# jbush001/RustNetworkStack

Measured on AMD Instinct MI355X. Metric: GiB/s device-resident Internet checksum, 1500B-packet batches, 1/2/4/8 GPUs, higher is better.
Workload: dtype u8

## Files before the change

include/rns_checksum.h:

```cpp
#ifndef RNS_CHECKSUM_H
#define RNS_CHECKSUM_H

#include <stddef.h>
#include <stdint.h>

#ifdef __cplusplus
extern "C" {
#endif

#define RNS_ABI_VERSION 1

#define RNS_OK            0
#define RNS_E_INVALID    (-1)
#define RNS_E_EMPTY      (-2)
#define RNS_E_BOUNDS     (-3)
#define RNS_E_NODEVICE   (-4)
#define RNS_E_ORDER      (-5)
#define RNS_E_TOOLARGE   (-6)
#define RNS_E_IO         (-7)
#define RNS_E_HIP_BASE   (-1000)

#define RNS_FLAG_COMPLEMENT 0x1u
#define RNS_FLAG_CHAIN_RUNS 0x2u
#define RNS_FLAG_CHAIN_TX_PACKED 0x4u

typedef struct rns_iovec {
    const uint8_t *base;
    size_t len;
} rns_iovec;

typedef struct rns_ipaddr {
    uint32_t version;
    uint8_t bytes[16];
} rns_ipaddr;


int32_t rns_compute_ones_comp(uint16_t in_checksum, const uint8_t *slice, size_t len);

int32_t rns_compute_checksum(const uint8_t *slice, size_t len);

int32_t rns_compute_buffer_ones_comp(uint16_t initial_sum, const rns_iovec *frags, size_t nfrags);

int32_t rns_compute_pseudo_header_checksum(const rns_ipaddr *source_ip, const rns_ipaddr *dest_ip,
                                           uint64_t length, uint8_t protocol);


int rns_csum_batch_dev(const uint8_t *d_arena, uint64_t arena_bytes, const uint64_t *d_off,
                       const uint32_t *d_len, const uint16_t *d_seed, uint16_t *d_out, uint32_t n,
                       uint32_t flags, uint32_t len_hint, uint32_t *d_bad, void *stream);

int rns_csum_batch_dev_off32(const uint8_t *d_arena, uint64_t arena_bytes, const uint32_t *d_off32,
                             const uint32_t *d_len, const uint16_t *d_seed, uint16_t *d_out, uint32_t n,
                             uint32_t flags, uint32_t len_hint, uint32_t *d_bad, void *stream);

int rns_csum_batch_packed_dev(const uint8_t *d_arena, uint64_t arena_bytes, const uint64_t *d_blk_off,
                              const uint16_t *d_len16, uint32_t align_log2, const uint16_t *d_seed, uint16_t *d_out,
                              uint32_t n, uint32_t flags, uint32_t len_hint, uint32_t *d_bad, void *stream);

int rns_packed_layout(const uint16_t *len16, uint64_t n, uint32_t align_log2, uint64_t first_off, uint64_t *blk_off,
                      uint64_t *off, uint64_t *end);

int rns_csum_batch_strided_dev(const uint8_t *d_arena, uint64_t arena_bytes, uint64_t first_off,
                               uint64_t stride, uint32_t len, const uint16_t *d_seed, uint16_t *d_out,
                               uint32_t n, uint32_t flags, uint32_t *d_bad, void *stream);

#define RNS_CHAIN_MAX_PACKETS (0xFFFFFFFFu - 512u)
int rns_csum_chain_dev(const uint8_t *d_arena, uint64_t arena_bytes, const uint64_t *d_frag_off,
                       const uint32_t *d_frag_len, uint32_t n_frags, const uint32_t *d_first,
                       const uint16_t *d_seed, uint16_t *d_out, uint32_t n_pkts, uint32_t flags,
                       uint32_t frag_len_hint, uint16_t *d_frag_sums, uint32_t *d_bad, void *stream);

int rns_csum_chain_fill_dev(uint8_t *d_arena, uint64_t arena_bytes, const uint64_t *d_frag_off,
                            const uint32_t *d_frag_len, uint32_t n_frags, const uint32_t *d_first,
                            const uint16_t *d_seed, const uint16_t *d_field, uint32_t field_off, uint16_t *d_out,
                            uint32_t n_pkts, uint32_t flags, uint32_t frag_len_hint, uint32_t *d_bad, void *stream);

int rns_csum_fill_dev(uint8_t *d_arena, uint64_t arena_bytes, const uint64_t *d_off, const uint32_t *d_len,
                      const uint16_t *d_seed, const uint16_t *d_field, uint32_t field_off, uint16_t *d_out,
                      uint32_t n, uint32_t flags, uint32_t *d_bad, void *stream);

int rns_csum_fill_packed_dev(uint8_t *d_arena, uint64_t arena_bytes, const uint64_t *d_blk_off, const uint16_t *d_len16,
                             uint32_t align_log2, const uint16_t *d_seed, const uint16_t *d_field, uint32_t field_off,
                             uint16_t *d_out, uint32_t n, uint32_t flags, uint32_t len_hint, uint32_t *d_bad,
                             void *stream);

#define RNS_RX_IP_OK          0x01u
#define RNS_RX_L4_OK          0x02u
#define RNS_RX_L4_UNCHECKED   0x04u
#define RNS_RX_FRAGMENT       0x08u
#define RNS_RX_UNKNOWN_PROTO  0x10u
#define RNS_RX_ACCEPT         0x40u
#define RNS_RX_MALFORMED      0x80u
int rns_rx_verify_dev(const uint8_t *d_arena, uint64_t arena_bytes, const uint64_t *d_off, const uint32_t *d_len,
                      uint32_t n, const uint8_t *local_ipv4, const uint8_t *local_ipv6, uint8_t *d_status,
                      uint16_t *d_l4_sum, void *stream);

int rns_rx_verify_packed_dev(const uint8_t *d_arena, uint64_t arena_bytes, const uint64_t *d_blk_off,
                             const uint16_t *d_len16, uint32_t align_log2, uint32_t n, const uint8_t *local_ipv4,
                             const uint8_t *local_ipv6, uint8_t *d_status, uint16_t *d_l4_sum, void *stream);

int rns_rx_verify_strided_dev(const uint8_t *d_arena, uint64_t arena_bytes, uint64_t first_off, uint64_t stride,
                              const uint16_t *d_len16, uint32_t n, const uint8_t *local_ipv4, const uint8_t *local_ipv6,
                              uint8_t *d_status, uint16_t *d_l4_sum, void *stream);

#define RNS_TX_IP_FILLED      0x01u
#define RNS_TX_L4_FILLED      0x02u
// ... 84 lines not shown
```

rustnetworkstack_amd/_lib.py:

```python
from __future__ import annotations

import ctypes
import os
import threading

PKG_DIR = os.path.dirname(os.path.abspath(__file__))
LIB_PATH = os.environ.get("RNS_CHECKSUM_LIB") or os.path.join(PKG_DIR, "librns_checksum.so")

RNS_OK = 0
RNS_E_INVALID = -1
RNS_E_EMPTY = -2
RNS_E_BOUNDS = -3
RNS_E_NODEVICE = -4
RNS_E_ORDER = -5
RNS_E_TOOLARGE = -6
RNS_E_IO = -7
RNS_E_HIP_BASE = -1000
RNS_FLAG_COMPLEMENT = 0x1
RNS_FLAG_CHAIN_RUNS = 0x2
RNS_FLAG_CHAIN_TX_PACKED = 0x4
RNS_CHAIN_MAX_PACKETS = 0xFFFFFFFF - 512
RNS_IO_MAX_FRAGS = 8
RNS_RX_IP_OK = 0x01
RNS_RX_L4_OK = 0x02
RNS_RX_L4_UNCHECKED = 0x04
RNS_RX_FRAGMENT = 0x08
RNS_RX_UNKNOWN_PROTO = 0x10
RNS_RX_ACCEPT = 0x40
RNS_RX_MALFORMED = 0x80
RNS_TX_IP_FILLED = 0x01
RNS_TX_L4_FILLED = 0x02
RNS_TX_MALFORMED = 0x80

EXPORTED_SYMBOLS = (
    "rns_compute_ones_comp",
    "rns_compute_checksum",
    "rns_compute_buffer_ones_comp",
    "rns_compute_pseudo_header_checksum",
    "rns_csum_batch_dev",
    "rns_csum_batch_dev_off32",
    "rns_csum_batch_packed_dev",
    "rns_packed_layout",
    "rns_csum_batch_strided_dev",
    "rns_csum_batch_dev_cfg",
    "rns_csum_chain_dev",
    "rns_csum_chain_fill_dev",
    "rns_csum_fill_dev",
    "rns_csum_fill_packed_dev",
    "rns_rx_verify_dev",
    "rns_rx_verify_packed_dev",
    "rns_rx_verify_strided_dev",
    "rns_tx_fill_dev",
    "rns_tx_fill_packed_dev",
    "rns_tx_fill_chain_dev",
    "rns_tx_fill_chain_packed_dev",
    "rns_tx_chain_packed_layout",
    "rns_host_ctx_create",
    "rns_host_ctx_destroy",
    "rns_csum_batch_host",
    "rns_multi_ctx_create",
    "rns_multi_ctx_destroy",
    "rns_csum_batch_multi_host",
    "rns_csum_batch_multi_dev",
    "rns_io_recv_batch",
    "rns_io_send_batch",
    "rns_io_send_batch_chain",
    "rns_io_recv_batch_packed",
    "rns_host_alloc",
    "rns_host_free",
    "rns_fill_splitmix64_dev",
    "rns_abi_version",
    "rns_strerror",
    "rns_build_info",
    "rns_csum_shape_name",
    "rns_device_count",
)


class ChecksumLibraryMissing(RuntimeError):
    """librns_checksum.so is not built: run __graft_entry__.build() (or `make`)."""


class ChecksumError(RuntimeError):
    def __init__(self, status: int, what: str):
        self.status = status
        super().__init__(f"{what}: {strerror(status)} (status {status})")


class RnsIovec(ctypes.Structure):
    _fields_ = [("base", ctypes.c_void_p), ("len", ctypes.c_size_t)]


class RnsIpAddr(ctypes.Structure):
    _fields_ = [("version", ctypes.c_uint32), ("bytes", ctypes.c_uint8 * 16)]


class RnsDevBatch(ctypes.Structure):
    _fields_ = [("device", ctypes.c_int), ("d_arena", ctypes.c_void_p), ("arena_bytes", ctypes.c_uint64),
                ("d_off", ctypes.c_void_p), ("d_len", ctypes.c_void_p), ("d_seed", ctypes.c_void_p),
                ("d_out", ctypes.c_void_p), ("n", ctypes.c_uint32), ("len_hint", ctypes.c_uint32),
                ("d_bad", ctypes.c_void_p), ("stream", ctypes.c_void_p)]


_LIB = None
_LOCK = threading.Lock()

_vp, _u8, _u16, _u32, _u64, _i32, _int, _sz = (
    ctypes.c_void_p, ctypes.c_uint8, ctypes.c_uint16, ctypes.c_uint32, ctypes.c_uint64,
    ctypes.c_int32, ctypes.c_int, ctypes.c_size_t)

_SIGNATURES = {
    "rns_compute_ones_comp": (_i32, [_u16, _vp, _sz]),
    "rns_compute_checksum": (_i32, [_vp, _sz]),
    "rns_compute_buffer_ones_comp": (_i32, [_u16, ctypes.POINTER(RnsIovec), _sz]),
    "rns_compute_pseudo_header_checksum": (_i32, [ctypes.POINTER(RnsIpAddr), ctypes.POINTER(RnsIpAddr), _u64, _u8]),
    "rns_csum_batch_dev": (_int, [_vp, _u64, _vp, _vp, _vp, _vp, _u32, _u32, _u32, _vp, _vp]),
    "rns_csum_batch_dev_off32": (_int, [_vp, _u64, _vp, _vp, _vp, _vp, _u32, _u32, _u32, _vp, _vp]),
    "rns_csum_batch_packed_dev": (_int, [_vp, _u64, _vp, _vp, _u32, _vp, _vp, _u32, _u32, _u32, _vp, _vp]),
    "rns_packed_layout": (_int, [_vp, _u64, _u32, _u64, _vp, _vp, ctypes.POINTER(_u64)]),
    "rns_csum_batch_strided_dev": (_int, [_vp, _u64, _u64, _u64, _u32, _vp, _vp, _u32, _u32, _vp, _vp]),
    "rns_csum_batch_dev_cfg": (_int, [_vp, _u64, _vp, _vp, _vp, _vp, _u32, _u32, _u32, _u32, _u32, _u32, _vp, _vp]),
    "rns_csum_chain_dev": (_int, [_vp, _u64, _vp, _vp, _u32, _vp, _vp, _vp, _u32, _u32, _u32, _vp, _vp, _vp]),
    "rns_csum_chain_fill_dev": (_int, [_vp, _u64, _vp, _vp, _u32, _vp, _vp, _vp, _u32, _vp, _u32, _u32, _u32, _vp,
                                       _vp]),
    "rns_csum_fill_dev": (_int, [_vp, _u64, _vp, _vp, _vp, _vp, _u32, _vp, _u32, _u32, _vp, _vp]),
    "rns_csum_fill_packed_dev": (_int, [_vp, _u64, _vp, _vp, _u32, _vp, _vp, _u32, _vp, _u32, _u32, _u32, _vp, _vp]),
    "rns_rx_verify_dev": (_int, [_vp, _u64, _vp, _vp, _u32, _vp, _vp, _vp, _vp, _vp]),
    "rns_rx_verify_packed_dev": (_int, [_vp, _u64, _vp, _vp, _u32, _u32, _vp, _vp, _vp, _vp, _vp]),
    "rns_rx_verify_strided_dev": (_int, [_vp, _u64, _u64, _u64, _vp, _u32, _vp, _vp, _vp, _vp, _vp]),
    "rns_tx_fill_dev": (_int, [_vp, _u64, _vp, _vp, _u32, _vp, _vp]),
    "rns_tx_fill_packed_dev": (_int, [_vp, _u64, _vp, _vp, _u32, _u32, _vp, _u32, _vp]),
    "rns_tx_fill_chain_dev": (_int, [_vp, _u64, _vp, _vp, _u32, _vp, _u32, _vp, _vp]),
    "rns_tx_fill_chain_packed_dev": (_int, [_vp, _u64, _vp, _vp, _vp, _vp, _u32, _u32, _vp, _vp]),
    "rns_tx_chain_packed_layout": (_int, [_vp, _vp, _u64, _u32, _u64, _u64, _vp, _vp, _vp, _vp,
                                          ctypes.POINTER(_u64), ctypes.POINTER(_u64)]),
    "rns_host_ctx_create": (_int, [_int, _u64, _u32, ctypes.POINTER(_vp)]),
    "rns_host_ctx_destroy": (_int, [_vp]),
    "rns_csum_batch_host": (_int, [_vp, _vp, _u64, _vp, _vp, _vp, _vp, _u32, _u32]),
    "rns_multi_ctx_create": (_int, [ctypes.POINTER(ctypes.c_int), _u32, _u64, _u32, ctypes.POINTER(_vp)]),
    "rns_multi_ctx_destroy": (_int, [_vp]),
    "rns_csum_batch_multi_host": (_int, [_vp, _vp, _u64, _vp, _vp, _vp, _vp, _u32, _u32]),
    "rns_csum_batch_multi_dev": (_int, [ctypes.POINTER(RnsDevBatch), _u32, _u32]),
    "rns_io_recv_batch": (_int, [_int, _vp, _u64, _u32, _vp, _vp, _int]),
    "rns_io_send_batch": (_int, [_int, _vp, _vp, _vp, _u32]),
    "rns_io_send_batch_chain": (_int, [_int, _vp, _vp, _vp, _vp, _u32]),
    "rns_io_recv_batch_packed": (_int, [_int, _vp, _u64, _u32, _u32, _vp, _vp, ctypes.POINTER(_u64), _int]),
    "rns_host_alloc": (_int, [_u64, ctypes.POINTER(_vp)]),
    "rns_host_free": (_int, [_vp]),
    "rns_fill_splitmix64_dev": (_int, [_vp, _u64, _u64, _vp]),
    "rns_abi_version": (_int, []),
    "rns_strerror": (ctypes.c_char_p, [_int]),
    "rns_build_info": (ctypes.c_char_p, []),
    "rns_csum_shape_name": (ctypes.c_char_p, [_u32]),
    "rns_device_count": (_int, []),
}


def load() -> ctypes.CDLL:
    global _LIB
    with _LOCK:
        if _LIB is None:
            try:
                import torch
            except ImportError:
                pass
            if not os.path.exists(LIB_PATH):
                raise ChecksumLibraryMissing(f"{LIB_PATH} not found; run __graft_entry__.build()")
            lib = ctypes.CDLL(LIB_PATH)
            for name, (res, args) in _SIGNATURES.items():
                fn = getattr(lib, name)
# ... 17 lines not shown
```

rustnetworkstack_amd/batch.py:

```python
from __future__ import annotations

import ctypes

import numpy as np
import torch

from . import _lib


def _require_cuda(t: torch.Tensor, name: str, dtypes) -> None:
    if not isinstance(t, torch.Tensor):
        raise TypeError(f"{name} must be a torch.Tensor")
    if t.device.type != "cuda":
        raise ValueError(f"{name} must be on a GPU device (got {t.device}); there is no CPU fallback")
    if t.dtype not in dtypes:
        raise TypeError(f"{name} dtype {t.dtype} not in {dtypes}")
    if not t.is_contiguous():
        raise ValueError(f"{name} must be contiguous")


_U16 = (torch.uint16, torch.int16)


def _rx_outputs(dev: torch.device, n: int, status, l4_sum, inputs):
# ... 125 lines not shown
        seed_ptr = None
        if seed is not None:
            _require_cuda(seed, "seed", _U16)
            if seed.numel() != n or seed.device != dev:
                raise ValueError("seed must have one entry per packet on the arena's device")
            seed_ptr = seed.data_ptr()
        if out is None:
            out = torch.empty(n, dtype=torch.uint16, device=dev)
        else:
            _require_cuda(out, "out", _U16)
            if out.numel() != n or out.device != dev:
                raise ValueError("out must have one entry per packet on the arena's device")
        bad_ptr = _bad_ptr(bad, arena.device)
        lib = _lib.load()
        self._keep = (arena, blk_off, len16, seed, out, bad)
        self.out, self.n, self.device = out, n, dev
        self._fn = lib.rns_csum_batch_packed_dev
        self._args = (arena.data_ptr(), arena.numel(), blk_off.data_ptr(), len16.data_ptr(), int(align_log2),
                      seed_ptr, out.data_ptr(), n, _lib.RNS_FLAG_COMPLEMENT if complement else 0, int(len_hint),
                      bad_ptr, _stream_handle(dev))

    def __call__(self) -> torch.Tensor:
        if self.n:
            if torch.cuda.current_device() != self.device.index:
                with torch.cuda.device(self.device):
                    st = self._fn(*self._args)
            else:
                st = self._fn(*self._args)
            if st != _lib.RNS_OK:
                raise _lib.ChecksumError(st, "rns_csum_batch_packed_dev")
        return self.out


def csum_batch_packed(arena: torch.Tensor, blk_off: torch.Tensor, len16: torch.Tensor,
                      seed: torch.Tensor | None = None, *, align_log2: int = 4, complement: bool = False,
                      out: torch.Tensor | None = None, len_hint: int = 0,
                      bad: torch.Tensor | None = None) -> torch.Tensor:
    _require_cuda(arena, "arena", (torch.uint8,))
    with torch.cuda.device(arena.device):
        return PackedBatch(arena, blk_off, len16, seed, align_log2=align_log2, complement=complement, out=out,
                           len_hint=len_hint, bad=bad)()


def csum_batch(arena: torch.Tensor, off: torch.Tensor, length: torch.Tensor, seed: torch.Tensor | None = None,
               *, complement: bool = False, out: torch.Tensor | None = None, len_hint: int = 0,
               bad: torch.Tensor | None = None, shape: tuple[int, int, int, int] | None = None,
               compact: bool = False) -> torch.Tensor:
    _require_cuda(arena, "arena", (torch.uint8,))
    with torch.cuda.device(arena.device):
        return PreparedBatch(arena, off, length, seed, complement=complement, out=out, len_hint=len_hint, bad=bad,
                             shape=shape, compact=compact)()


class StridedBatch:

    def __init__(self, arena: torch.Tensor, n: int, stride: int, length: int, *, first_off: int = 0,
                 seed: torch.Tensor | None = None, complement: bool = False,
                 out: torch.Tensor | None = None, bad: torch.Tensor | None = None):
        _require_cuda(arena, "arena", (torch.uint8,))
        dev = arena.device
        if n < 0 or n >= 2 ** 32 or stride < 0 or not 0 <= length < 2 ** 32 or first_off < 0:
            raise ValueError("n, stride, length and first_off must be non-negative (n, length < 2^32)")
        seed_ptr = None
        if seed is not None:
            _require_cuda(seed, "seed", _U16)
            if seed.numel() != n or seed.device != dev:
                raise ValueError("seed must have one entry per packet on the arena's device")
            seed_ptr = seed.data_ptr()
        if out is None:
            out = torch.empty(n, dtype=torch.uint16, device=dev)
        else:
            _require_cuda(out, "out", _U16)
            if out.numel() != n or out.device != dev:
                raise ValueError("out must have one entry per packet on the arena's device")
        bad_ptr = _bad_ptr(bad, arena.device)
        lib = _lib.load()
        self._keep = (arena, seed, out, bad)
        self.out, self.n, self.device = out, int(n), dev
        self._fn = lib.rns_csum_batch_strided_dev
        self._args = (arena.data_ptr(), arena.numel(), int(first_off), int(stride), int(length), seed_ptr,
                      out.data_ptr(), int(n), _lib.RNS_FLAG_COMPLEMENT if complement else 0, bad_ptr,
                      _stream_handle(dev))

    def __call__(self) -> torch.Tensor:
        if self.n:
            if torch.cuda.current_device() != self.device.index:
                with torch.cuda.device(self.device):
                    st = self._fn(*self._args)
            else:
                st = self._fn(*self._args)
            if st != _lib.RNS_OK:
                raise _lib.ChecksumError(st, "rns_csum_batch_strided_dev")
        return self.out


def csum_batch_strided(arena: torch.Tensor, n: int, stride: int, length: int, *, first_off: int = 0,
                       seed: torch.Tensor | None = None, complement: bool = False,
                       out: torch.Tensor | None = None, bad: torch.Tensor | None = None) -> torch.Tensor:
    _require_cuda(arena, "arena", (torch.uint8,))
    with torch.cuda.device(arena.device):
        return StridedBatch(arena, n, stride, length, first_off=first_off, seed=seed, complement=complement,
                            out=out, bad=bad)()


def csum_chain(arena: torch.Tensor, frag_off: torch.Tensor, frag_len: torch.Tensor, first: torch.Tensor,
               seed: torch.Tensor | None = None, *, complement: bool = False, out: torch.Tensor | None = None,
# ... 557 lines not shown
```

rustnetworkstack_amd/csrc/k_packed.hip:

```cpp
#include "rns_launch.hpp"

#ifndef RNS_ROWS_DEEP_FROM
#define RNS_ROWS_DEEP_FROM 1024u
#endif

namespace rns {

#ifndef RNS_RX_ROWS_D
#define RNS_RX_ROWS_D 8
#endif
int launch_stream_rx(const CsumArgs &a, hipStream_t st)
{
    const dim3 grid(static_cast<uint32_t>((static_cast<uint64_t>(a.n) + 63) / 64)), block(64);
    constexpr bool NT = RNS_STREAM_NT != 0;
    const bool ack = a.arena_bytes / a.n <= 128, buf = buf_records(a) < kOobOffset;
    if (ack && buf)
        hipLaunchKernelGGL((csum_stream_kernel<NT, true>), grid, block, 0, st, a);
    else if (ack)
        hipLaunchKernelGGL((csum_stream_kernel<NT, false>), grid, block, 0, st, a);
    else if (buf)
        hipLaunchKernelGGL((csum_rows_rx_kernel<NT, true, RNS_RX_ROWS_D>), grid, block, 0, st, a);
    else
        hipLaunchKernelGGL((csum_rows_rx_kernel<NT, false, RNS_RX_ROWS_D>), grid, block, 0, st, a);
    return hip_status(hipGetLastError());
}

int dispatch_packed(const CsumArgs &a, const Shape &sh, hipStream_t st)
{
    const bool nt = (sh.variant & 2u) != 0, buf = buf_records(a) < kOobOffset;
    const bool tiny = (sh.variant & ~16u) == 3u && sh.G == 4u && sh.U == 1u;
    if (a.align_mask >= 15u && !tiny) {
        constexpr bool NT = RNS_STREAM_NT != 0;
        const dim3 grid(static_cast<uint32_t>((static_cast<uint64_t>(a.n) + 63) / 64)), block(64);
        if (a.len_hint >= RNS_ROWS_DEEP_FROM) {
            if (buf)
                hipLaunchKernelGGL((csum_rows_kernel<NT, true, 16>), grid, block, 0, st, a);
            else
                hipLaunchKernelGGL((csum_rows_kernel<NT, false, 16>), grid, block, 0, st, a);
        } else {
            if (buf)
                hipLaunchKernelGGL((csum_rows_kernel<NT, true, 8>), grid, block, 0, st, a);
            else
                hipLaunchKernelGGL((csum_rows_kernel<NT, false, 8>), grid, block, 0, st, a);
        }
        return hip_status(hipGetLastError());
    }
    const uint64_t batches = (static_cast<uint64_t>(a.n) + 63) / 64;
    const uint64_t wpb = ((sh.variant & 4u) ? kMixedBlock<false> : kBlock) / 64;
    uint64_t blocks = (batches + wpb - 1) / wpb;
    if (sh.max_blocks != 0 && blocks > sh.max_blocks)
        blocks = sh.max_blocks;
    const dim3 grid(static_cast<uint32_t>(blocks)), block((sh.variant & 4u) ? kMixedBlock<false> : kBlock);
    if (sh.variant & 4u) {
        if (nt && buf)
            hipLaunchKernelGGL((csum_mixed_kernel<false, true, true, false, false, false, true>), grid, block, 0, st, a);
        else if (nt)
            hipLaunchKernelGGL((csum_mixed_kernel<false, true, false, false, false, false, true>), grid, block, 0, st, a);
// ... 76 lines not shown
```

rustnetworkstack_amd/csrc/rns_checksum.hip:

```cpp
#include <hip/hip_runtime.h>

#include <algorithm>
#include <cmath>
#include <cstdint>
#include <cstdio>
#include <cstring>
#include <mutex>
#include <new>
#include <thread>
#include <vector>

#include "rns_launch.hpp"

using namespace rns;

namespace {

__global__ __launch_bounds__(kBlock) void splitmix64_fill_kernel(uint8_t *buf, uint64_t nbytes, uint64_t seed)
{
    const uint64_t nwords = (nbytes + 7) / 8;
    const uint64_t stride = static_cast<uint64_t>(gridDim.x) * blockDim.x;
    for (uint64_t i = static_cast<uint64_t>(blockIdx.x) * blockDim.x + threadIdx.x; i < nwords; i += stride) {
        uint64_t z = seed + (i + 1) * 0x9E3779B97F4A7C15ull;
        z = (z ^ (z >> 30)) * 0xBF58476D1CE4E5B9ull;
// ... 21 lines not shown
        uint16_t *d_out = nullptr;
        uint64_t *h_off = nullptr;
        uint32_t *h_len = nullptr;
        uint16_t *h_seed = nullptr;
        uint16_t *h_out = nullptr;
        bool busy = false;
        uint32_t i0 = 0, cnt = 0;
    };
    int device = 0;
    uint64_t chunk_bytes = 0;
    uint32_t chunk_packets = 0;
    std::vector<Slot> slots;
    std::mutex mu;
};

namespace {

void free_ctx(rns_host_ctx *c)
{
    if (!c)
        return;
    (void)hipSetDevice(c->device);
    for (auto &s : c->slots) {
        if (s.stream) (void)hipStreamSynchronize(s.stream);
        if (s.done) (void)hipEventDestroy(s.done);
        if (s.stream) (void)hipStreamDestroy(s.stream);
        (void)hipFree(s.d_arena); (void)hipFree(s.d_off); (void)hipFree(s.d_len);
        (void)hipFree(s.d_seed); (void)hipFree(s.d_out);
        (void)hipHostFree(s.h_off); (void)hipHostFree(s.h_len);
        (void)hipHostFree(s.h_seed); (void)hipHostFree(s.h_out);
    }
    delete c;
}

int drain_slot(rns_host_ctx::Slot &s, uint16_t *h_out)
{
    if (!s.busy)
        return RNS_OK;
    s.busy = false;
    int st = hip_status(hipEventSynchronize(s.done));
    if (st == RNS_OK)
        std::memcpy(h_out + s.i0, s.h_out, static_cast<size_t>(s.cnt) * sizeof(uint16_t));
    return st;
}

}

static bool strided_fits(uint64_t first_off, uint64_t stride, uint32_t n)
{
    const uint64_t room = ~0ull - 16u - first_off;
    return first_off <= ~0ull - 16u && (n <= 1 || stride <= room / (n - 1));
}

extern "C" {

int rns_csum_batch_dev_cfg(const uint8_t *d_arena, uint64_t arena_bytes, const uint64_t *d_off,
                           const uint32_t *d_len, const uint16_t *d_seed, uint16_t *d_out, uint32_t n,
                           uint32_t flags, uint32_t variant, uint32_t lanes_per_packet, uint32_t unroll,
                           uint32_t max_blocks, uint32_t *d_bad, void *stream)
{
    if (n == 0)
        return RNS_OK;
    if (!d_arena || !d_off || !d_len || !d_out)
        return RNS_E_INVALID;
    if (int st = check_device())
        return st;
    CsumArgs a{};
    set_arena(a, d_arena, arena_bytes);
    a.off = d_off;
    a.len = d_len;
    a.seed = d_seed;
    a.out = d_out;
    a.bad = d_bad;
    a.n = n;
    a.flags = flags;
    return dispatch<false>(a, variant, lanes_per_packet, unroll, max_blocks, static_cast<hipStream_t>(stream));
}

int rns_csum_batch_dev(const uint8_t *d_arena, uint64_t arena_bytes, const uint64_t *d_off,
                       const uint32_t *d_len, const uint16_t *d_seed, uint16_t *d_out, uint32_t n,
                       uint32_t flags, uint32_t len_hint, uint32_t *d_bad, void *stream)
{
    const Shape sh = pick_shape(len_hint);
    return rns_csum_batch_dev_cfg(d_arena, arena_bytes, d_off, d_len, d_seed, d_out, n, flags, sh.variant, sh.G,
                                  sh.U, sh.max_blocks, d_bad, stream);
}

int rns_csum_batch_dev_off32(const uint8_t *d_arena, uint64_t arena_bytes, const uint32_t *d_off32,
                             const uint32_t *d_len, const uint16_t *d_seed, uint16_t *d_out, uint32_t n,
                             uint32_t flags, uint32_t len_hint, uint32_t *d_bad, void *stream)
{
    if (n == 0)
        return RNS_OK;
    if (!d_arena || !d_off32 || !d_len || !d_out)
        return RNS_E_INVALID;
    if (int st = check_device())
        return st;
    const Shape sh = pick_shape(len_hint);
    CsumArgs a{};
    set_arena(a, d_arena, arena_bytes);
    a.off32 = d_off32;
    a.len = d_len;
    a.seed = d_seed;
    a.out = d_out;
    a.bad = d_bad;
    a.n = n;
    a.flags = flags;
    return dispatch<false>(a, sh.variant, sh.G, sh.U, sh.max_blocks, static_cast<hipStream_t>(stream));
}

int rns_csum_batch_packed_dev(const uint8_t *d_arena, uint64_t arena_bytes, const uint64_t *d_blk_off,
                              const uint16_t *d_len16, uint32_t align_log2, const uint16_t *d_seed, uint16_t *d_out,
                              uint32_t n, uint32_t flags, uint32_t len_hint, uint32_t *d_bad, void *stream)
{
    if (n == 0)
        return RNS_OK;
    if (!d_arena || !d_blk_off || !d_len16 || !d_out || align_log2 > 12)
        return RNS_E_INVALID;
    if (int st = check_device())
        return st;
    Shape sh = pick_shape(len_hint);
    if ((sh.variant & 5u) == 0)
        sh = Shape{6u, 0u, 0u, 0u};

    CsumArgs a{};
    set_arena(a, d_arena, arena_bytes);
    a.len16 = d_len16;
    a.blk_off = d_blk_off;
    a.align_mask = (1u << align_log2) - 1u;
    a.seed = d_seed;
    a.out = d_out;
    a.bad = d_bad;
    a.n = n;
    a.flags = flags;
    a.len_hint = len_hint;
    return dispatch_packed(a, sh, static_cast<hipStream_t>(stream));
}

int rns_csum_batch_strided_dev(const uint8_t *d_arena, uint64_t arena_bytes, uint64_t first_off,
                               uint64_t stride, uint32_t len, const uint16_t *d_seed, uint16_t *d_out,
                               uint32_t n, uint32_t flags, uint32_t *d_bad, void *stream)
{
    if (n == 0)
        return RNS_OK;
    if (!d_arena || !d_out || !strided_fits(first_off, stride, n))
        return RNS_E_INVALID;
    if (int st = check_device())
        return st;
    CsumArgs a{};
    set_arena(a, d_arena, arena_bytes);
    a.seed = d_seed;
    a.out = d_out;
    a.bad = d_bad;
    a.first_off = first_off;
    a.stride = stride;
    a.fixed_len = len;
    a.n = n;
    a.flags = flags;
    if (len != 0 && len <= 64 && ((first_off + a.base_adjust) & 15) == 0 && (stride & 15) == 0)
        return launch_strided_tiny(a, static_cast<hipStream_t>(stream));
    const Shape sh = pick_shape(len);
// ... 548 lines not shown
    if (nbatches == 0)
        return RNS_OK;
    if (!batches)
        return RNS_E_INVALID;
    if (int st = check_device())
        return st;
    int prev = 0;
    if (hipGetDevice(&prev) != hipSuccess)
        return RNS_E_NODEVICE;
    int st = RNS_OK;
    for (uint32_t k = 0; k < nbatches && st == RNS_OK; ++k) {
        const rns_dev_batch &d = batches[k];
        st = hip_status(hipSetDevice(d.device));
        if (st == RNS_OK)
            st = rns_csum_batch_dev(d.d_arena, d.arena_bytes, d.d_off, d.d_len, d.d_seed, d.d_out, d.n, flags,
                                    d.len_hint, d.d_bad, d.stream);
    }
    (void)hipSetDevice(prev);
    return st;
}

int rns_host_alloc(uint64_t bytes, void **out)
{
    if (!out)
        return RNS_E_INVALID;
    *out = nullptr;
    if (int st = check_device())
        return st;
    return hip_status(hipHostMalloc(out, bytes, 0));
}

int rns_host_free(void *p) { return hip_status(hipHostFree(p)); }

int rns_fill_splitmix64_dev(uint8_t *d_buf, uint64_t nbytes, uint64_t seed, void *stream)
{
    if (nbytes == 0)
        return RNS_OK;
    if (!d_buf || (reinterpret_cast<uintptr_t>(d_buf) & 7))
        return RNS_E_INVALID;
    if (int st = check_device())
        return st;
    const uint64_t words = (nbytes + 7) / 8;
    const uint32_t blocks = static_cast<uint32_t>(std::min<uint64_t>((words + kBlock - 1) / kBlock, 8192));
    hipLaunchKernelGGL(splitmix64_fill_kernel, dim3(blocks), dim3(kBlock), 0, static_cast<hipStream_t>(stream),
                       d_buf, nbytes, seed);
    return hip_status(hipGetLastError());
}

const char *rns_csum_shape_name(uint32_t len_hint)
{
    static const char *const names[] = {"csum_batch_kernel",     "csum_rounds_kernel",     "csum_batch_kernel[nt]",
                                        "csum_rounds_kernel[nt]", "csum_mixed_kernel",      "csum_mixed_kernel",
                                        "csum_mixed_kernel[nt]",  "csum_mixed_kernel[nt]"};
    static thread_local char buf[96];
    const Shape sh = pick_shape(len_hint);
    if (sh.variant & 4)
        std::snprintf(buf, sizeof(buf), "%s (size classes G/U 4/1 x 4 packets, 4/4, 16/4, 32/4, 64/4)", names[sh.variant & 7]);
    else
        std::snprintf(buf, sizeof(buf), "%s<G=%u,U=%u>%s%s", names[sh.variant & 7], sh.G, sh.U,
                      (sh.variant & 8) ? " all rounds in flight" : (sh.variant & 16) ? " descriptors prefetched" : "",
                      sh.max_blocks ? " grid-capped" : "");
    return buf;
}

const char *rns_build_info(void)
{
    return "rns_checksum abi=1 offload-arch=gfx950 kernels=csum_rows_kernel (packed form: 1 KiB rows per 64-packet "
           "region, owners capture two region prefixes and sum their own end chunk; fill mode), csum_rows_rx_kernel "
           "(packed receive verify: the rows plus each owner's header chunks loaded a group ahead), csum_stream_kernel "
           "(receive verify of ACK-sized arenas: owners load their datagrams whole), csum_strided_rx_kernel (receive "
           "verify of fixed-size slots: quad-coalesced rows), csum_rows_tx_kernel (packed transmit finalize through the "
           "rows), csum_txrows_kernel (transmit-shaped chains: packed payload rows + owner-loaded head fragments; "
           "head-fragment fill; whole finalize of NetBuffer chains with the heads written back from LDS), "
           "csum_strided_tiny_kernel "
           "(fixed-size packets <= 64 B at a fixed stride), csum_mixed_kernel (per-wave size-class sort; verify / fill / "
           "transmit-finalize stash modes), csum_rounds_kernel, csum_batch_kernel, csum_chain_kernel (one pass, "
           "per-fragment fold; head-fragment fill) (v_sad_u16 LE sums, v_dot4 BE sums past 128 KiB, wave64, DPP "
           "reductions)";
}

int rns_device_count(void)
{
    int n = 0;
    if (hipGetDeviceCount(&n) != hipSuccess) {
        (void)hipGetLastError();
        return 0;
    }
    return n;
}

}
```

rustnetworkstack_amd/csrc/rns_k_common.hpp:

```cpp
#pragma once

#include <hip/hip_runtime.h>

#include <algorithm>
#include <cmath>
#include <cstdint>
#include <cstdio>
#include <cstring>
#include <mutex>
#include <new>
#include <thread>
#include <type_traits>
#include <vector>

#include "rns_checksum.h"

namespace rns {

#ifndef RNS_BLOCK
#define RNS_BLOCK 256
#endif
constexpr int kBlock = RNS_BLOCK;

struct CsumArgs {
    const uint8_t *arena;
    uint64_t arena_bytes;
    uint64_t base_adjust;
    const uint64_t *off;
    const uint32_t *off32;
    const uint32_t *len;
    const uint16_t *seed;
    uint16_t *out;
    uint32_t *bad;
    uint64_t first_off;
    uint64_t stride;
    uint32_t fixed_len;
    uint32_t n;
    uint32_t flags;
    const uint16_t *field;
    uint32_t field_off;
    uint8_t *status;
    uint16_t *l4_out;
    uint32_t local4_sum;
    uint32_t local6_sum;
    const uint16_t *len16;
    const uint64_t *blk_off;
    uint32_t align_mask;
    const uint32_t *first;
    uint32_t n_frags;
    uint32_t chain_k;
    uint32_t len_hint;
    const uint8_t *head_len8;
    const uint64_t *head_blk_off;
};

typedef unsigned int u32x4 __attribute__((ext_vector_type(4)));

__device__ __forceinline__ uint64_t desc_off(const CsumArgs &a, uint64_t p)
{
    return a.off32 ? static_cast<uint64_t>(a.off32[p]) : a.off[p];
}

template <int CTRL, int ROW_MASK = 0xF, int BANK_MASK = 0xF>
__device__ __forceinline__ uint32_t dpp_or_zero(uint32_t v)
{
    return static_cast<uint32_t>(
        __builtin_amdgcn_update_dpp(0, static_cast<int>(v), CTRL, ROW_MASK, BANK_MASK, true));
}

__device__ __forceinline__ uint32_t wave_excl_scan(uint32_t v)
{
    uint32_t x = v;
    x += dpp_or_zero<0x111>(v);
    x += dpp_or_zero<0x112>(v);
    x += dpp_or_zero<0x113>(v);
    x += dpp_or_zero<0x114, 0xF, 0xE>(x);
    x += dpp_or_zero<0x118, 0xF, 0xC>(x);
    x += dpp_or_zero<0x142, 0xA, 0xF>(x);
    x += dpp_or_zero<0x143, 0xC, 0xF>(x);
    return x - v;
}

__device__ __forceinline__ uint32_t packed_scan(const CsumArgs &a, uint32_t lane, uint32_t len)
{
    (void)lane;
    const uint32_t pad = (len + a.align_mask) & ~a.align_mask;
    return wave_excl_scan(pad);
}

__device__ __forceinline__ uint64_t packed_off(const CsumArgs &a, uint64_t base, uint32_t lane, uint32_t len)
{
    return a.blk_off[base >> 6] + packed_scan(a, lane, len);
}

#ifndef RNS_NT_AUX
#define RNS_NT_AUX 2
#endif
constexpr int kNtAux = RNS_NT_AUX;

template <bool NT>
__device__ __forceinline__ uint4 load_chunk(const uint8_t *p)
{
    if constexpr (NT) {
        const u32x4 v = __builtin_nontemporal_load(reinterpret_cast<const u32x4 *>(p));
        return make_uint4(v.x, v.y, v.z, v.w);
    } else {
// ... 109 lines not shown
```

rustnetworkstack_amd/csrc/rns_kernels.hpp:

```cpp
#pragma once

#include "rns_k_common.hpp"
#include "rns_k_rounds.hpp"
#include "rns_k_mixed.hpp"
#include "rns_k_chain.hpp"
#include "rns_k_stream.hpp"
#include "rns_k_rows.hpp"
```

rustnetworkstack_amd/csrc/rns_launch.hpp:

```cpp
#pragma once

#include "rns_kernels.hpp"

namespace rns {

inline int hip_status(hipError_t e) { return e == hipSuccess ? RNS_OK : RNS_E_HIP_BASE - static_cast<int>(e); }

struct Shape {
    uint32_t variant, G, U, max_blocks;
};

constexpr uint32_t kTinyVariant = 19u;
constexpr uint32_t kTinyGrid = 2048u;
inline Shape pick_shape(uint32_t len_hint)
{
    const uint32_t chunks = len_hint ? (len_hint + 15) / 16 + 1 : 96;
    if (chunks <= 8)
        return Shape{kTinyVariant, 4u, 1u, kTinyGrid};
    if (chunks <= 48)
        return Shape{4u, 0u, 0u, 0u};
    if (chunks <= 160)
        return Shape{6u, 0u, 0u, 0u};
    return Shape{2u, 64u, 4u, 0u};
}

inline int check_device()
{
    int n = 0;
    if (hipGetDeviceCount(&n) != hipSuccess || n <= 0) {
        (void)hipGetLastError();
        return RNS_E_NODEVICE;
    }
    return RNS_OK;
}

inline void set_arena(CsumArgs &a, const uint8_t *arena, uint64_t arena_bytes)
{
    const uintptr_t p = reinterpret_cast<uintptr_t>(arena);
    a.base_adjust = p & 15;
    a.arena = reinterpret_cast<const uint8_t *>(p - a.base_adjust);
    a.arena_bytes = arena_bytes + a.base_adjust;
}


template <bool S>
int dispatch(const CsumArgs &a, uint32_t variant, uint32_t G, uint32_t U, uint32_t max_blocks, hipStream_t st);
extern template int dispatch<false>(const CsumArgs &, uint32_t, uint32_t, uint32_t, uint32_t, hipStream_t);
extern template int dispatch<true>(const CsumArgs &, uint32_t, uint32_t, uint32_t, uint32_t, hipStream_t);
int launch_strided_tiny(const CsumArgs &a, hipStream_t st);
int dispatch_packed(const CsumArgs &a, const Shape &sh, hipStream_t st);
int launch_fill_packed(const CsumArgs &a, hipStream_t st);
int launch_stream_rx(const CsumArgs &a, hipStream_t st);
int launch_tx_packed(const CsumArgs &a, hipStream_t st);
int launch_strided_rx(const CsumArgs &a, hipStream_t st);
template <bool FILL>
int launch_chain(const CsumArgs &a, uint32_t K, bool nt, bool runs, hipStream_t st);
extern template int launch_chain<false>(const CsumArgs &, uint32_t, bool, bool, hipStream_t);
extern template int launch_chain<true>(const CsumArgs &, uint32_t, bool, bool, hipStream_t);
template <bool FILL>
int launch_txrows(const CsumArgs &a, hipStream_t st);
extern template int launch_txrows<false>(const CsumArgs &, hipStream_t);
extern template int launch_txrows<true>(const CsumArgs &, hipStream_t);
int launch_txfin(const CsumArgs &a, hipStream_t st);
int launch_txfin_packed(const CsumArgs &a, hipStream_t st);
int launch_fill(const CsumArgs &a, dim3 grid, hipStream_t st);
int launch_rx(const CsumArgs &a, dim3 grid, hipStream_t st);
int launch_tx(const CsumArgs &a, dim3 grid, hipStream_t st);

}
```

Baseline: 6720.

## Route explicit-descriptor batches through region row streaming when packets are contiguous

Adds a rows-explicit kernel for the explicit-offset batch entry points. Each wave checks whether its 64 descriptors form an ascending, 16-byte-aligned, densely packed region. If so, it streams that region as 1 KiB rows, reusing the packed-layout row summation. Other waves fall back to the size-class pass. The per-wave ballot and scan setup adds overhead, and irregular layouts see no benefit. A diagnostic entry point counts slow-path waves.

```diff
diff --git a/include/rns_checksum.h b/include/rns_checksum.h
--- a/include/rns_checksum.h
+++ b/include/rns_checksum.h
@@ -52,6 +52,11 @@
 int rns_csum_batch_dev_off32(const uint8_t *d_arena, uint64_t arena_bytes, const uint32_t *d_off32,
                              const uint32_t *d_len, const uint16_t *d_seed, uint16_t *d_out, uint32_t n,
                              uint32_t flags, uint32_t len_hint, uint32_t *d_bad, void *stream);
+
+int rns_csum_batch_dev_diag(const uint8_t *d_arena, uint64_t arena_bytes, const uint64_t *d_off,
+                            const uint32_t *d_off32, const uint32_t *d_len, const uint16_t *d_seed, uint16_t *d_out,
+                            uint32_t n, uint32_t flags, uint32_t len_hint, uint32_t *d_bad,
+                            uint32_t *d_slow_waves, void *stream);
 
 int rns_csum_batch_packed_dev(const uint8_t *d_arena, uint64_t arena_bytes, const uint64_t *d_blk_off,
                               const uint16_t *d_len16, uint32_t align_log2, const uint16_t *d_seed, uint16_t *d_out,
diff --git a/rustnetworkstack_amd/_lib.py b/rustnetworkstack_amd/_lib.py
--- a/rustnetworkstack_amd/_lib.py
+++ b/rustnetworkstack_amd/_lib.py
@@ -39,6 +39,7 @@
     "rns_compute_pseudo_header_checksum",
     "rns_csum_batch_dev",
     "rns_csum_batch_dev_off32",
+    "rns_csum_batch_dev_diag",
     "rns_csum_batch_packed_dev",
     "rns_packed_layout",
     "rns_csum_batch_strided_dev",
@@ -116,6 +117,7 @@
     "rns_compute_pseudo_header_checksum": (_i32, [ctypes.POINTER(RnsIpAddr), ctypes.POINTER(RnsIpAddr), _u64, _u8]),
     "rns_csum_batch_dev": (_int, [_vp, _u64, _vp, _vp, _vp, _vp, _u32, _u32, _u32, _vp, _vp]),
     "rns_csum_batch_dev_off32": (_int, [_vp, _u64, _vp, _vp, _vp, _vp, _u32, _u32, _u32, _vp, _vp]),
+    "rns_csum_batch_dev_diag": (_int, [_vp, _u64, _vp, _vp, _vp, _vp, _vp, _u32, _u32, _u32, _vp, _vp, _vp]),
     "rns_csum_batch_packed_dev": (_int, [_vp, _u64, _vp, _vp, _u32, _vp, _vp, _u32, _u32, _u32, _vp, _vp]),
     "rns_packed_layout": (_int, [_vp, _u64, _u32, _u64, _vp, _vp, ctypes.POINTER(_u64)]),
     "rns_csum_batch_strided_dev": (_int, [_vp, _u64, _u64, _u64, _u32, _vp, _vp, _u32, _u32, _vp, _vp]),
diff --git a/rustnetworkstack_amd/batch.py b/rustnetworkstack_amd/batch.py
--- a/rustnetworkstack_amd/batch.py
+++ b/rustnetworkstack_amd/batch.py
@@ -201,6 +201,40 @@
                              shape=shape, compact=compact)()
 
 
+def csum_batch_diag(arena: torch.Tensor, off: torch.Tensor, length: torch.Tensor, seed: torch.Tensor | None = None,
+                    *, slow_waves: torch.Tensor, complement: bool = False, out: torch.Tensor | None = None,
+                    len_hint: int = 0, bad: torch.Tensor | None = None, compact: bool = False) -> torch.Tensor:
+    _require_cuda(arena, "arena", (torch.uint8,))
+    _require_cuda(off, "off", (torch.int32,) if compact else (torch.int64,))
+    _require_cuda(length, "length", (torch.int32,))
+    n = off.numel()
+    if length.numel() != n or n >= 2 ** 32:
+        raise ValueError("off and length must have the same number of packets (below 2^32)")
+    dev = arena.device
+    for name, t in (("off", off), ("length", length)):
+        if t.device != dev:
+            raise ValueError(f"{name} is on {t.device}, arena on {dev}")
+    seed_ptr = None
+    if seed is not None:
+        _require_cuda(seed, "seed", _U16)
+        if seed.numel() != n or seed.device != dev:
+            raise ValueError("seed must have one entry per packet on the arena's device")
+        seed_ptr = seed.data_ptr()
+    if out is None:
+        out = torch.empty(n, dtype=torch.uint16, device=dev)
+    else:
+        _require_cuda(out, "out", _U16)
+        if out.numel() != n or out.device != dev:
+            raise ValueError("out must have one entry per packet on the arena's device")
+    with torch.cuda.device(dev):
+        st = _lib.load().rns_csum_batch_dev_diag(
+            arena.data_ptr(), arena.numel(), None if compact else off.data_ptr(), off.data_ptr() if compact else None,
+            length.data_ptr(), seed_ptr, out.data_ptr(), n, _lib.RNS_FLAG_COMPLEMENT if complement else 0,
+            int(len_hint), _bad_ptr(bad, dev), _bad_ptr(slow_waves, dev), _stream_handle(dev))
+    _lib.check(st, "rns_csum_batch_dev_diag")
+    return out
+
+
 class StridedBatch:
 
     def __init__(self, arena: torch.Tensor, n: int, stride: int, length: int, *, first_off: int = 0,
diff --git a/rustnetworkstack_amd/csrc/k_packed.hip b/rustnetworkstack_amd/csrc/k_packed.hip
--- a/rustnetworkstack_amd/csrc/k_packed.hip
+++ b/rustnetworkstack_amd/csrc/k_packed.hip
@@ -1,8 +1,4 @@
 #include "rns_launch.hpp"
-
-#ifndef RNS_ROWS_DEEP_FROM
-#define RNS_ROWS_DEEP_FROM 1024u
-#endif
 
 namespace rns {
 
diff --git a/rustnetworkstack_amd/csrc/k_rows_explicit.hip b/rustnetworkstack_amd/csrc/k_rows_explicit.hip
--- /dev/null
+++ b/rustnetworkstack_amd/csrc/k_rows_explicit.hip
@@ -0,0 +1,36 @@
+#include "rns_launch.hpp"
+
+namespace rns {
+
+template <bool BUF, bool OFF32>
+static void launch_rows_explicit_d(const CsumArgs &a, dim3 grid, hipStream_t st)
+{
+    constexpr bool NT = RNS_STREAM_NT != 0;
+    static_assert(RNS_ROWS_DEEP_FROM > 752u, "every D = 16 hint takes the nontemporal class pass");
+    if (a.len_hint >= RNS_ROWS_DEEP_FROM)
+        hipLaunchKernelGGL((csum_rows_explicit_kernel<NT, BUF, 16, OFF32, true>), grid, dim3(64), 0, st, a);
+    else if (pick_shape(a.len_hint).variant & 2u)
+        hipLaunchKernelGGL((csum_rows_explicit_kernel<NT, BUF, 8, OFF32, true>), grid, dim3(64), 0, st, a);
+    else
+        hipLaunchKernelGGL((csum_rows_explicit_kernel<NT, BUF, 8, OFF32, false>), grid, dim3(64), 0, st, a);
+}
+
+int launch_rows_explicit(const CsumArgs &a, hipStream_t st)
+{
+    const dim3 grid(static_cast<uint32_t>((static_cast<uint64_t>(a.n) + 63) / 64));
+    const bool buf = buf_records(a) < kOobOffset;
+    if (a.off32) {
+        if (buf)
+            launch_rows_explicit_d<true, true>(a, grid, st);
+        else
+            launch_rows_explicit_d<false, true>(a, grid, st);
+    } else {
+        if (buf)
+            launch_rows_explicit_d<true, false>(a, grid, st);
+        else
+            launch_rows_explicit_d<false, false>(a, grid, st);
+    }
+    return hip_status(hipGetLastError());
+}
+
+}
diff --git a/rustnetworkstack_amd/csrc/rns_checksum.hip b/rustnetworkstack_amd/csrc/rns_checksum.hip
--- a/rustnetworkstack_amd/csrc/rns_checksum.hip
+++ b/rustnetworkstack_amd/csrc/rns_checksum.hip
@@ -97,6 +97,35 @@
     return first_off <= ~0ull - 16u && (n <= 1 || stride <= room / (n - 1));
 }
 
+static int batch_explicit(const uint8_t *d_arena, uint64_t arena_bytes, const uint64_t *d_off,
+                          const uint32_t *d_off32, const uint32_t *d_len, const uint16_t *d_seed, uint16_t *d_out,
+                          uint32_t n, uint32_t flags, uint32_t len_hint, uint32_t *d_bad, uint32_t *d_slow_waves,
+                          void *stream)
+{
+    if (n == 0)
+        return RNS_OK;
+    if (!d_arena || (!d_off && !d_off32) || !d_len || !d_out)
+        return RNS_E_INVALID;
+    if (int st = check_device())
+        return st;
+    CsumArgs a{};
+    set_arena(a, d_arena, arena_bytes);
+    a.off = d_off32 ? nullptr : d_off;
+    a.off32 = d_off32;
+    a.len = d_len;
+    a.seed = d_seed;
+    a.out = d_out;
+    a.bad = d_bad;
+    a.n = n;
+    a.flags = flags;
+    a.len_hint = len_hint;
+    a.slow_waves = d_slow_waves;
+    if (rows_hint(len_hint))
+        return launch_rows_explicit(a, static_cast<hipStream_t>(stream));
+    const Shape sh = pick_shape(len_hint);
+    return dispatch<false>(a, sh.variant, sh.G, sh.U, sh.max_blocks, static_cast<hipStream_t>(stream));
+}
+
 extern "C" {
 
 int rns_csum_batch_dev_cfg(const uint8_t *d_arena, uint64_t arena_bytes, const uint64_t *d_off,
@@ -126,32 +155,29 @@
                        const uint32_t *d_len, const uint16_t *d_seed, uint16_t *d_out, uint32_t n,
                        uint32_t flags, uint32_t len_hint, uint32_t *d_bad, void *stream)
 {
-    const Shape sh = pick_shape(len_hint);
-    return rns_csum_batch_dev_cfg(d_arena, arena_bytes, d_off, d_len, d_seed, d_out, n, flags, sh.variant, sh.G,
-                                  sh.U, sh.max_blocks, d_bad, stream);
+    if (n != 0 && !d_off)
+        return RNS_E_INVALID;
+    return batch_explicit(d_arena, arena_bytes, d_off, nullptr, d_len, d_seed, d_out, n, flags, len_hint, d_bad,
+                          nullptr, stream);
+}
+
+int rns_csum_batch_dev_diag(const uint8_t *d_arena, uint64_t arena_bytes, const uint64_t *d_off,
+                            const uint32_t *d_off32, const uint32_t *d_len, const uint16_t *d_seed, uint16_t *d_out,
+                            uint32_t n, uint32_t flags, uint32_t len_hint, uint32_t *d_bad,
+                            uint32_t *d_slow_waves, void *stream)
+{
+    return batch_explicit(d_arena, arena_bytes, d_off, d_off32, d_len, d_seed, d_out, n, flags, len_hint, d_bad,
+                          d_slow_waves, stream);
 }
 
 int rns_csum_batch_dev_off32(const uint8_t *d_arena, uint64_t arena_bytes, const uint32_t *d_off32,
                              const uint32_t *d_len, const uint16_t *d_seed, uint16_t *d_out, uint32_t n,
                              uint32_t flags, uint32_t len_hint, uint32_t *d_bad, void *stream)
 {
-    if (n == 0)
-        return RNS_OK;
-    if (!d_arena || !d_off32 || !d_len || !d_out)
-        return RNS_E_INVALID;
-    if (int st = check_device())
-        return st;
-    const Shape sh = pick_shape(len_hint);
-    CsumArgs a{};
-    set_arena(a, d_arena, arena_bytes);
-    a.off32 = d_off32;
-    a.len = d_len;
-    a.seed = d_seed;
-    a.out = d_out;
-    a.bad = d_bad;
-    a.n = n;
-    a.flags = flags;
-    return dispatch<false>(a, sh.variant, sh.G, sh.U, sh.max_blocks, static_cast<hipStream_t>(stream));
+    if (n != 0 && !d_off32)
+        return RNS_E_INVALID;
+    return batch_explicit(d_arena, arena_bytes, nullptr, d_off32, d_len, d_seed, d_out, n, flags, len_hint, d_bad,
+                          nullptr, stream);
 }
 
 int rns_csum_batch_packed_dev(const uint8_t *d_arena, uint64_t arena_bytes, const uint64_t *d_blk_off,
@@ -806,10 +832,13 @@
     static const char *const names[] = {"csum_batch_kernel",     "csum_rounds_kernel",     "csum_batch_kernel[nt]",
                                         "csum_rounds_kernel[nt]", "csum_mixed_kernel",      "csum_mixed_kernel",
                                         "csum_mixed_kernel[nt]",  "csum_mixed_kernel[nt]"};
-    static thread_local char buf[96];
+    static thread_local char buf[256];
     const Shape sh = pick_shape(len_hint);
-    if (sh.variant & 4)
-        std::snprintf(buf, sizeof(buf), "%s (size classes G/U 4/1 x 4 packets, 4/4, 16/4, 32/4, 64/4)", names[sh.variant & 7]);
+    if (rows_hint(len_hint))
+        std::snprintf(buf, sizeof(buf),
+                      "csum_rows_explicit_kernel<D=%d> (a wave whose 64 descriptors form a region streams it as 1 KiB "
+                      "rows; any other wave: the class pass, size classes G/U 4/1 x 4 packets, 4/4, 16/4, 32/4, 64/4)",
+                      len_hint >= RNS_ROWS_DEEP_FROM ? 16 : 8);
     else
         std::snprintf(buf, sizeof(buf), "%s<G=%u,U=%u>%s%s", names[sh.variant & 7], sh.G, sh.U,
                       (sh.variant & 8) ? " all rounds in flight" : (sh.variant & 16) ? " descriptors prefetched" : "",
@@ -820,7 +849,9 @@
 const char *rns_build_info(void)
 {
     return "rns_checksum abi=1 offload-arch=gfx950 kernels=csum_rows_kernel (packed form: 1 KiB rows per 64-packet "
-           "region, owners capture two region prefixes and sum their own end chunk; fill mode), csum_rows_rx_kernel "
+           "region, owners capture two region prefixes and sum their own end chunk; fill mode), "
+           "csum_rows_explicit_kernel (explicit descriptors: the same rows for every wave whose 64 packets form a "
+           "region, the class pass for the others), csum_rows_rx_kernel "
            "(packed receive verify: the rows plus each owner's header chunks loaded a group ahead), csum_stream_kernel "
            "(receive verify of ACK-sized arenas: owners load their datagrams whole), csum_strided_rx_kernel (receive "
            "verify of fixed-size slots: quad-coalesced rows), csum_rows_tx_kernel (packed transmit finalize through the "
diff --git a/rustnetworkstack_amd/csrc/rns_k_common.hpp b/rustnetworkstack_amd/csrc/rns_k_common.hpp
--- a/rustnetworkstack_amd/csrc/rns_k_common.hpp
+++ b/rustnetworkstack_amd/csrc/rns_k_common.hpp
@@ -52,6 +52,7 @@
     uint32_t len_hint;
     const uint8_t *head_len8;
     const uint64_t *head_blk_off;
+    uint32_t *slow_waves;
 };
 
 typedef unsigned int u32x4 __attribute__((ext_vector_type(4)));
diff --git a/rustnetworkstack_amd/csrc/rns_k_rows_explicit.hpp b/rustnetworkstack_amd/csrc/rns_k_rows_explicit.hpp
--- /dev/null
+++ b/rustnetworkstack_amd/csrc/rns_k_rows_explicit.hpp
@@ -0,0 +1,96 @@
+#pragma once
+
+#include "rns_k_rows.hpp"
+
+namespace rns {
+
+struct RowsRegion {
+    uint64_t r0;
+    uint32_t total;
+    uint32_t c0, e;
+    bool fast;
+};
+
+__device__ __forceinline__ RowsRegion explicit_rows_region(uint64_t start, uint32_t len, bool has, uint32_t lane)
+{
+    RowsRegion g{0, 0, 0, 0, true};
+    const uint64_t pm = __ballot(has);
+    if (!pm)
+        return g;
+    g.r0 = lane_u64(start, static_cast<uint32_t>(__builtin_ctzll(pm)));
+    const uint64_t rel64 = has ? start - g.r0 : 0;
+    const bool fits = !has || (rel64 < (1ull << 30) && (start & 15u) == 0 && len <= 0xFFFFu);
+    const uint32_t rel = static_cast<uint32_t>(rel64);
+    const uint32_t pad = has && fits ? (len + 15u) & ~15u : 0u;
+    const uint32_t end = has && fits ? rel + pad : 0u;
+    const uint32_t incl = wave_incl_max(end);
+    const uint32_t before = static_cast<uint32_t>(__shfl(static_cast<int>(incl), static_cast<int>(lane) - 1, 64));
+    const bool asc = !has || (fits && (lane == 0 || rel >= before));
+    g.total = __builtin_amdgcn_readlane(incl, 63);
+    const uint32_t sum_pad = __builtin_amdgcn_readlane(wave_incl_scan(pad), 63);
+    g.fast = !__ballot(!asc) && g.total <= 2u * sum_pad + 4096u;
+    g.c0 = has ? rel >> 4 : 0u;
+    g.e = has ? (rel + len - 1u) >> 4 : 0u;
+    return g;
+}
+
+#ifndef RNS_ROWS_EXPLICIT_OCC
+#define RNS_ROWS_EXPLICIT_OCC 4
+#endif
+
+template <bool NT, bool BUF, int D, bool OFF32, bool CNT = NT>
+__global__ __launch_bounds__(64, D >= 16 ? 4 : RNS_ROWS_EXPLICIT_OCC) void csum_rows_explicit_kernel(const CsumArgs a)
+{
+    const uint32_t lane = threadIdx.x;
+    const __amdgpu_buffer_rsrc_t rsrc = __builtin_amdgcn_make_buffer_rsrc(
+        const_cast<uint8_t *>(a.arena), static_cast<short>(0), static_cast<int>(BUF ? buf_records(a) : 0), 0x00020000);
+    const uint64_t recs = buf_records(a);
+    const uint64_t p = static_cast<uint64_t>(blockIdx.x) * 64 + lane;
+    const bool live = p < a.n;
+    const uint64_t q = live ? p : a.n - 1;
+    uint64_t off;
+    if constexpr (OFF32)
+        off = a.off32[q];
+    else
+        off = a.off[q];
+    const uint32_t len = live ? a.len[q] : 0u;
+    const uint32_t seed = (a.seed && live) ? static_cast<uint32_t>(a.seed[q]) : 0u;
+    if constexpr (BUF && !OFF32)
+        off = off > 0xFFFFFFFFull ? 0xFFFFFFFFull : off;
+    const uint64_t start = (live ? off : 0) + a.base_adjust;
+    const bool ok = start <= a.arena_bytes && len <= a.arena_bytes - start;
+    const bool has = live && ok && len != 0;
+    const RowsRegion g = explicit_rows_region(start, len, has, lane);
+    if (g.fast) {
+        const uint32_t mine = rows_region_sum<NT, BUF, D>(a, rsrc, recs, g.r0, g.total, g.c0, g.e, has ? len : 0u);
+        const uint16_t res = finalize_bits(mine, false, false, seed, ok, a.flags);
+        if (live) {
+            if (a.n < (1u << 30)) {
+                const __amdgpu_buffer_rsrc_t out_rsrc = __builtin_amdgcn_make_buffer_rsrc(
+                    static_cast<void *>(a.out), static_cast<short>(0), static_cast<int>(2u * a.n), 0x00020000);
+                __builtin_amdgcn_raw_buffer_store_b16(res, out_rsrc, static_cast<uint32_t>(2 * p), 0, RNS_STREAM_OUT_AUX);
+            } else {
+                __builtin_nontemporal_store(res, a.out + p);
+            }
+        }
+    } else {
+        if (a.slow_waves && lane == 0)
+            atomicAdd(a.slow_waves, 1u);
+        const uint64_t d_start = has ? start : 0;
+        const uint32_t d_len = has ? len : 0u;
+        const bool odd = d_start & 1, big = d_len > kNoWrapBytes;
+        uint32_t pos;
+        const uint32_t mine =
+            wave_class_pass<CNT, BUF, kStashNone>(a, rsrc, d_start, d_len, 0xFFFFFFFFu, lane, nullptr, pos);
+        const uint16_t res = finalize_bits(mine, odd, big, seed, ok, a.flags);
+        if (live)
+            __builtin_nontemporal_store(res, a.out + p);
+    }
+    if (a.bad) {
+        const uint64_t rejected = __ballot(live && !ok);
+        if (rejected && lane == 0)
+            atomicAdd(a.bad, static_cast<uint32_t>(__popcll(rejected)));
+    }
+}
+
+}
diff --git a/rustnetworkstack_amd/csrc/rns_kernels.hpp b/rustnetworkstack_amd/csrc/rns_kernels.hpp
--- a/rustnetworkstack_amd/csrc/rns_kernels.hpp
+++ b/rustnetworkstack_amd/csrc/rns_kernels.hpp
@@ -6,3 +6,4 @@
 #include "rns_k_chain.hpp"
 #include "rns_k_stream.hpp"
 #include "rns_k_rows.hpp"
+#include "rns_k_rows_explicit.hpp"
diff --git a/rustnetworkstack_amd/csrc/rns_launch.hpp b/rustnetworkstack_amd/csrc/rns_launch.hpp
--- a/rustnetworkstack_amd/csrc/rns_launch.hpp
+++ b/rustnetworkstack_amd/csrc/rns_launch.hpp
@@ -24,6 +24,12 @@
     return Shape{2u, 64u, 4u, 0u};
 }
 
+#ifndef RNS_ROWS_DEEP_FROM
+#define RNS_ROWS_DEEP_FROM 1024u
+#endif
+
+inline bool rows_hint(uint32_t len_hint) { return pick_shape(len_hint).variant != kTinyVariant; }
+
 inline int check_device()
 {
     int n = 0;
@@ -48,6 +54,7 @@
 extern template int dispatch<false>(const CsumArgs &, uint32_t, uint32_t, uint32_t, uint32_t, hipStream_t);
 extern template int dispatch<true>(const CsumArgs &, uint32_t, uint32_t, uint32_t, uint32_t, hipStream_t);
 int launch_strided_tiny(const CsumArgs &a, hipStream_t st);
+int launch_rows_explicit(const CsumArgs &a, hipStream_t st);
 int dispatch_packed(const CsumArgs &a, const Shape &sh, hipStream_t st);
 int launch_fill_packed(const CsumArgs &a, hipStream_t st);
 int launch_stream_rx(const CsumArgs &a, hipStream_t st);
```

Result: no change. 6714 (median of 2 runs) (-0.1%).
